# MIT-SPARK/Hydra-GNN

Hardware: AMD Instinct MI355X
Metric: scene-graphs/sec (fwd+bwd) MP3D hetero batch (higher is better)
Workload: dtype f32

## Files before the change

hydra-gnn_amd/csrc/gemm.hip:

```cpp
#include <algorithm>

#include "gemm_tile.h"

namespace hmp {

KT_DEFINE(gemm)

template <int ROWS, int BK>
using TileSide = TileSlots<256, ROWS, BK>;
template <int ROWS, int BK>
using TileRegs = StageRegs<TileSide<ROWS, BK>::NV>;

template <int ROWS, int BK>
__device__ __forceinline__ void tile_load_edge(TileRegs<ROWS, BK>& t, const float* __restrict__ p, int ld, int kcontig, int r0,
                                               int R, int n_real, int aug, int k0, int kend, int vec) {
  using S = TileSide<ROWS, BK>;
#pragma unroll
  for (int i = 0; i < S::NV; ++i) {
    float4 val = make_float4(0.f, 0.f, 0.f, 0.f);
    if (kcontig) {
      int r, k4;
      S::slot_rk(i, r, k4);
      const int gr = r0 + r, gk = k0 + k4;
      if (gr < R && gk < kend) {
// ... 405 lines not shown
    P.M = g.M; P.N = g.N; P.K = g.K; P.lda = g.lda; P.ldb = g.ldb; P.ldc = g.ldc; P.n_real = g.n_real; P.aug_ones = g.aug_ones;
    P.nslices = cdiv(g.N, TT_NS);
    int ks = (int)(512.0 * ((double)g.K * P.nslices / work_total) / P.nslices + 0.5);
    if (ks > GEMM_TALL_SLABS) ks = GEMM_TALL_SLABS;
    if (ks < 1) ks = 1;
    P.kchunk = g.kchunk = cdiv(cdiv(g.K, ks), TT_BK) * TT_BK;
    P.ksplit = g.ksplit = cdiv(g.K, P.kchunk);
    P.block_start = start;
    start += P.ksplit * P.nslices;
  }
  static const int rc = [] {
    return hipFuncSetAttribute(reinterpret_cast<const void*>(&gemm_tn_tall_kernel), hipFuncAttributeMaxDynamicSharedMemorySize,
                               2 * TT_STAGE * (int)sizeof(float)) == hipSuccess ? 0 : 1;
  }();
  HMP_CHECK_ARG(rc == 0, "gemm: could not raise the dynamic LDS limit of the tall weight-gradient kernel");
  hipLaunchKernelGGL(gemm_tn_tall_kernel, dim3(start), dim3(256), 2 * TT_STAGE * sizeof(float), st, tb);
  HMP_LAUNCH_CHECK();
  return HMP_OK;
}

int gemm_launch(GemmBatch& gb, bool want_split, int max_slabs, hipStream_t st) {
  HMP_CHECK_ARG(gb.n >= 0 && gb.n <= GEMM_MAX_PROB, "gemm: %d problems", gb.n);
  if (gemm_x3_takes(gb, want_split)) return gemm_x3_launch(gb, want_split, max_slabs, st);
  if (want_split) {
    GemmPeel tall;
    gemm_peel(gb, tall_takes, tall);
    if (tall.n_taken > 0) {
      HMP_TRY(tall_launch(gb, tall, st));
      return gemm_launch_rest(gb, tall, [&](GemmBatch& rest) { return gemm_launch(rest, want_split, max_slabs, st); });
    }
  }
  int64_t tiles64 = 0;
  double work = 0.0;
  int max_k = 0;
  for (int i = 0; i < gb.n; ++i) {
    const GemmProblem& p = gb.p[i];
    HMP_CHECK_ARG(p.M >= 0 && p.N >= 0 && p.K >= 0, "gemm: negative size");
    tiles64 += (int64_t)cdiv(p.M, 64) * cdiv(p.N, 64);
    work += (double)p.M * p.N * p.K;
    max_k = p.K > max_k ? p.K : max_k;
  }
  if (tiles64 >= 1024 || work >= 1e9) {
    int64_t tiles128 = 0;
    for (int i = 0; i < gb.n; ++i) tiles128 += (int64_t)cdiv(gb.p[i].M, 128) * cdiv(gb.p[i].N, 128);
    const bool big_ok = env_switch("HMP_GEMM_BIG") != '0';
    int min_n = 1 << 30;
    for (int i = 0; i < gb.n; ++i) min_n = gb.p[i].N < min_n ? gb.p[i].N : min_n;
    if (big_ok && min_n >= 256 && work >= 1e9 && (tiles128 >= 256 || (want_split && max_k >= 8192)))
      return launch_cfg<2, 2, 32, 2, 2>(gb, want_split, max_slabs, st);
    return launch_cfg<2, 2, 32>(gb, want_split, max_slabs, st);
  }
  if (max_k <= 64) return launch_cfg<1, 1, 64>(gb, want_split, max_slabs, st);
  return launch_cfg<1, 1, 128>(gb, want_split, max_slabs, st);
}

}

extern "C" int hmp_gemm_f32(const float* d_a, int32_t lda, int32_t trans_a, const float* d_b, int32_t ldb, int32_t trans_b,
                            float* d_c, int32_t ldc, int32_t M, int32_t N, int32_t K, void* stream) {
  using namespace hmp;
  HMP_CHECK_ARG(d_a && d_b && d_c, "hmp_gemm_f32: null pointer");
  HMP_CHECK_ARG(M >= 0 && N >= 0 && K >= 0, "hmp_gemm_f32: negative size");
  HMP_CHECK_ARG(lda >= (trans_a ? M : K) && ldb >= (trans_b ? K : N) && ldc >= N, "hmp_gemm_f32: leading dimension too small");
  GemmBatch gb;
  memset(&gb, 0, sizeof(gb));
  gb.n = 1;
  GemmProblem& p = gb.p[0];
  p.A = d_a; p.B = d_b; p.C = d_c;
  p.M = M; p.N = N; p.K = K;
  p.lda = lda; p.ldb = ldb; p.ldc = ldc;
  p.trans_a = trans_a; p.trans_b = trans_b;
  p.n_real = N;
  p.epi = EPI_NONE;
  if (M == 0 || N == 0) return HMP_OK;
  return gemm_launch(gb, false, 1, (hipStream_t)stream);
}

extern "C" int hmp_gemm_grouped(const hmp_gemm_desc* d, int32_t n, int32_t route, int32_t want_split, int32_t max_slabs,
                                int32_t* ksplit_out, void* stream) {
  using namespace hmp;
  static const bool have_device = hmp_device_count() > 0;
  HMP_CHECK_ARG(have_device, "hmp_gemm_grouped: no gfx950 device visible");
  HMP_CHECK_ARG((d || n == 0) && n >= 0 && n <= GEMM_MAX_PROB, "hmp_gemm_grouped: %d problems (at most %d)", n, GEMM_MAX_PROB);
  HMP_CHECK_ARG(route >= 0 && route <= 2 && max_slabs >= 1, "hmp_gemm_grouped: route %d, max_slabs %d", route, max_slabs);
  for (int i = 0; i < n; ++i) {
    const hmp_gemm_desc& q = d[i];
    HMP_CHECK_ARG(q.A && q.B && q.C, "hmp_gemm_grouped: null pointer (problem %d)", i);
    HMP_CHECK_ARG(q.M >= 0 && q.N >= 0 && q.K >= 0, "hmp_gemm_grouped: negative size (problem %d)", i);
    HMP_CHECK_ARG(q.n_real == q.N - (q.aug_ones ? 1 : 0) && q.n_real >= 0, "hmp_gemm_grouped: n_real %d, N %d, aug_ones %d (problem %d)",
                  q.n_real, q.N, q.aug_ones, i);
    HMP_CHECK_ARG(q.lda >= (q.trans_a ? q.M : q.K) && q.ldb >= (q.trans_b ? q.K : q.n_real) && q.ldc >= q.N,
                  "hmp_gemm_grouped: leading dimension too small (problem %d)", i);
    HMP_CHECK_ARG(q.epi == EPI_NONE || (q.epi == EPI_ACTMASK && q.H && q.ldh >= q.N), "hmp_gemm_grouped: epilogue (problem %d)", i);
    HMP_CHECK_ARG(!q.Cadd || q.ldadd >= q.N, "hmp_gemm_grouped: ldadd too small (problem %d)", i);
    HMP_CHECK_ARG(q.drop_p >= 0.f && q.drop_p < 1.f, "hmp_gemm_grouped: drop_p %g (problem %d)", (double)q.drop_p, i);
    HMP_CHECK_ARG(!want_split || q.M == 0 || q.slab_stride >= (int64_t)q.M * q.ldc, "hmp_gemm_grouped: slab_stride (problem %d)", i);
    HMP_CHECK_ARG(route == 1 || !(q.a_bf16 || q.b_bf16 || q.c_bf16 || q.h_bf16), "hmp_gemm_grouped: bf16 operands on route %d", route);
    HMP_CHECK_ARG(route != 2 || (q.trans_a && !q.trans_b && q.epi == EPI_NONE && !q.Cadd),
                  "hmp_gemm_grouped: the direct kernel takes the plain TN form only (problem %d)", i);
  }
  hipStream_t st = (hipStream_t)stream;
  if (route == 2) {
    TnBatch tb;
    memset(&tb, 0, sizeof(tb));
    tb.n = n;
    for (int i = 0; i < n; ++i) {
      const hmp_gemm_desc& q = d[i];
      TnProblem& P = tb.p[i];
      P.A = (const float*)q.A; P.B = (const float*)q.B; P.C = (float*)q.C; P.slab_stride = q.slab_stride;
      P.M = q.M; P.N = q.N; P.K = q.K; P.lda = q.lda; P.ldb = q.ldb; P.ldc = q.ldc;
      P.n_real = q.n_real; P.aug_ones = q.aug_ones;
    }
    int ok = 0;
    HMP_TRY(gemm_tn_direct_launch(tb, max_slabs, &ok, st));
    if (ksplit_out)
      for (int i = 0; i < n; ++i) ksplit_out[i] = ok ? tb.p[i].ksplit : 0;
    return HMP_OK;
  }
  GemmBatch gb;
  memset(&gb, 0, sizeof(gb));
  gb.n = n;
  for (int i = 0; i < n; ++i) {
    const hmp_gemm_desc& q = d[i];
    GemmProblem& p = gb.p[i];
    p.A = (const float*)q.A; p.B = (const float*)q.B; p.C = (float*)q.C; p.H = (const float*)q.H;
    p.a_bf16 = q.a_bf16; p.b_bf16 = q.b_bf16; p.c_bf16 = q.c_bf16; p.h_bf16 = q.h_bf16;
    p.slab_stride = q.slab_stride;
    p.M = q.M; p.N = q.N; p.K = q.K;
    p.lda = q.lda; p.ldb = q.ldb; p.ldc = q.ldc; p.ldh = q.ldh;
    p.trans_a = q.trans_a; p.trans_b = q.trans_b;
    p.n_real = q.n_real; p.aug_ones = q.aug_ones;
    p.epi = q.epi; p.act = q.act;
    p.drop_on = q.drop_p > 0.f ? 1 : 0;
    p.drop.thresh = drop_thresh(q.drop_p); p.drop.scale = 1.f / (1.f - q.drop_p);
    p.Cadd = q.Cadd; p.ldadd = q.ldadd;
  }
  const int rc = route == 0 ? gemm_launch(gb, want_split != 0, max_slabs, st) : gemm_bf16_launch(gb, want_split != 0, max_slabs, st);
  if (ksplit_out)
    for (int i = 0; i < n; ++i) ksplit_out[i] = gb.p[i].ksplit;
  return rc;
}
```

hydra-gnn_amd/csrc/gemm_direct.hip:

```cpp
#include "device_fns.h"

namespace hmp {

KT_DEFINE(gemmd)

typedef float f32x16 __attribute__((ext_vector_type(16)));

__device__ __forceinline__ void reduce4(f32x16& acc, float* red , int w, int lane, float (&out)[4]) {
#pragma unroll
  for (int i = 0; i < 16; ++i) red[(w * 16 + i) * 64 + lane] = acc[i];
  __syncthreads();
#pragma unroll
  for (int j = 0; j < 4; ++j) {
    const int i = 4 * w + j;
    out[j] = (red[(0 * 16 + i) * 64 + lane] + red[(1 * 16 + i) * 64 + lane]) + (red[(2 * 16 + i) * 64 + lane] + red[(3 * 16 + i) * 64 + lane]);
  }
}

constexpr int TN_MAXI = 24;

__global__ __launch_bounds__(256, 2) void gemm_tn_direct_kernel(const TnBatch tb) {
  __shared__ float red[4 * 16 * 64];
  const int blk = blockIdx.x;
  KT(8);
  karg_warm<(sizeof(TnBatch) + 63) / 64>(0, (int)sizeof(TnBatch));
  int pi = 0;
  while (pi + 1 < tb.n && blk >= tb.p[pi + 1].tile_start) ++pi;
  const TnProblem& P = tb.p[pi];
  const int local = blk - P.tile_start;
  const int z = local % P.ksplit, t = local / P.ksplit;
  const int tm = t / P.tiles_n, tn = t % P.tiles_n;
  const int m0 = tm * 32, n0 = tn * 32;
  const int lane = threadIdx.x & 63, w = threadIdx.x >> 6;
  const int r = lane & 31, h = lane >> 5;
  const int kbeg = z * P.kchunk, kend = min(P.K, kbeg + P.kchunk);
  const int n_steps = (kend - kbeg + 1) >> 1;
  const int per = (n_steps + 3) >> 2;
  const int s0 = w * per, s1 = min(n_steps, s0 + per);
  const int am = min(m0 + r, P.M - 1);
  const int bn = n0 + r;
  const bool b_real = bn < P.n_real;
  const bool b_one = P.aug_ones && bn == P.n_real;
  const int bnc = b_real ? bn : 0;
  f32x16 acc;
#pragma unroll
  for (int i = 0; i < 16; ++i) acc[i] = 0.f;
  for (int sb0 = s0; sb0 < s1; sb0 += TN_MAXI) {
    float av[TN_MAXI], bv[TN_MAXI];
#pragma unroll
    for (int i = 0; i < TN_MAXI; ++i) {
      const int k = kbeg + 2 * (sb0 + i) + h;
      const bool live = (sb0 + i < s1) && k < kend;
      const int kc = live ? k : kbeg;
      const float a = P.A[(int64_t)kc * P.lda + am];
      const float b = P.B[(int64_t)kc * P.ldb + bnc];
      av[i] = live ? a : 0.f;
      bv[i] = live ? (b_real ? b : (b_one ? 1.f : 0.f)) : 0.f;
    }
#pragma unroll
    for (int i = 0; i < TN_MAXI; ++i)
      if (sb0 + i < s1) acc = __builtin_amdgcn_mfma_f32_32x32x2f32(av[i], bv[i], acc, 0, 0, 0);
  }
  float out[4];
  reduce4(acc, red, w, lane, out);
  float* C = P.C + (int64_t)z * P.slab_stride;
  const int col = n0 + (lane & 31);
  if (col < P.N) {
#pragma unroll
    for (int j = 0; j < 4; ++j) {
      const int row = m0 + j + 8 * w + 4 * h;
      if (row < P.M) C[(int64_t)row * P.ldc + col] = out[j];
    }
  }
  KT(9);
}

int gemm_tn_direct_launch(TnBatch& tb, int max_slabs, int* ok, hipStream_t st) {
  int start = 0;
  *ok = 1;
  for (int i = 0; i < tb.n; ++i) {
    TnProblem& P = tb.p[i];
    P.tiles_m = cdiv(P.M, 32);
    P.tiles_n = cdiv(P.N, 32);
    const int trips = (P.tiles_m * P.tiles_n >= 512) ? 4 : 2;
    int ks = cdiv(P.K, 2 * 4 * TN_MAXI * trips);
    if (ks < 1) ks = 1;
    if (ks > max_slabs) { *ok = 0; return HMP_OK; }
    while (ks * 2 <= max_slabs && cdiv(P.K, ks * 2) >= 32 && P.tiles_m * P.tiles_n * ks < 256) ks *= 2;
    int kchunk = cdiv(cdiv(P.K, ks), 2) * 2;
    if (kchunk < 2) kchunk = 2;
    ks = P.K > 0 ? cdiv(P.K, kchunk) : 1;
    P.ksplit = ks;
    P.kchunk = kchunk;
    P.tile_start = start;
    start += P.tiles_m * P.tiles_n * ks;
  }
  tb.total_tiles = start;
  if (start == 0) return HMP_OK;
  hipLaunchKernelGGL(gemm_tn_direct_kernel, dim3(start), dim3(256), 0, st, tb);
  HMP_LAUNCH_CHECK();
  return HMP_OK;
}

}
```

hydra-gnn_amd/csrc/kernels.h:

```cpp
#pragma once
#include "common.h"

namespace hmp {

enum { EPI_NONE = 0, EPI_ACTMASK = 1 };

struct GemmProblem {
  const float* A;
  const float* B;
  float* C;
  const float* H;
  int c_bf16;
  int a_bf16;
  int b_bf16;
  int h_bf16;
  const float* A2;
  int lda2, a_split;
  int64_t slab_stride;
  int M, N, K;
  int lda, ldb, ldc, ldh;
  int trans_a;
  int trans_b;
  int n_real;
  int aug_ones;
// ... 83 lines not shown
    gb.p[s.rest_idx[i]].kchunk = s.rest.p[i].kchunk;
  }
  return rc;
}

struct XcdGrid {
  int groups, tiles_per_group;
};
inline XcdGrid xcd_set_grid(int per_cu, int n_slices, int n_tiles) {
  int sets = per_cu * device_cu_count() / (8 * n_slices);
  if (sets < 1) sets = 1;
  int groups = 8 * sets;
  if (groups > n_tiles) groups = ((n_tiles + 7) / 8) * 8;
  return {groups, cdiv(n_tiles, groups)};
}

int gemm_launch(GemmBatch& gb, bool want_split, int max_slabs, hipStream_t st);
int gemm_bf16_launch(GemmBatch& gb, bool want_split, int max_slabs, hipStream_t st);
bool gemm_x3_takes(const GemmBatch& gb, bool want_split);
bool gemm_x3_split_takes(const GemmProblem* ps, int n);
int gemm_x3_launch(GemmBatch& gb, bool want_split, int max_slabs, hipStream_t st);
bool gemm_bf16_dx_takes(const GemmProblem& p, bool want_split);
int gemm_bf16_dx_launch(const GemmProblem& p, hipStream_t st);
bool gemm_bf16_dw_takes(const GemmProblem& p, bool want_split);
int gemm_bf16_dw_launch(const GemmProblem& p, int max_slabs, int* n_slabs, hipStream_t st);

constexpr int FR_MAX_PROB = 4;
constexpr int FR_MAX_SEG = 6;
constexpr int FR_MAX_SRC = 6;
struct FrontSeg {
  int col0, rows, nsrc, ld;
  uint32_t off[FR_MAX_SRC];
};
struct FrontProb {
  const float* A;
  float* C;
  int lda, ldc, M, N, K;
  int n_seg, max_nsrc, vec;
  int blk_start, tiles_m, tiles_n;
  FrontSeg seg[FR_MAX_SEG];
};
struct FrontJob {
  const int64_t* ei;
  int E, n_src, n_dst;
  uint32_t rowptr, col, eid, t_rowptr, t_col, t_eid, tmp_in, tmp_out, pos_of_eid, degf;
  const int64_t *gp_dst, *gp_src, *gp_edge;
  int n_graphs;
};
struct PackSeg;
struct NetState;
struct FrontArgs {
  int gemm_blocks, plan_blocks, pack_blocks;
  int n_prob, n_jobs, need_tpos, plan_rc;
  const float* params;
  char* ws;
  int* status;
  const PackSeg* segs;
  const int2* pack_map;
  float* packed;
  int* step_ctr;
  int* step_mirror;
  int prob_start[FR_MAX_PROB];
  int part_start[2 * HMP_MAX_EDGE_TYPES + 1];
  int rows_per_part[2 * HMP_MAX_EDGE_TYPES];
  FrontJob job[HMP_MAX_EDGE_TYPES];
  FrontProb prob[FR_MAX_PROB];
};
int front_launch(FrontArgs& a, hipStream_t st);

struct TnProblem {
  const float* A;
  const float* B;
  float* C;
  int64_t slab_stride;
  int M, N, K, lda, ldb, ldc;
  int n_real, aug_ones;
  int ksplit, kchunk, tile_start, tiles_m, tiles_n;
};
struct TnBatch {
  int n, total_tiles;
  TnProblem p[GEMM_MAX_PROB];
};
int gemm_tn_direct_launch(TnBatch& tb, int max_slabs, int* ok, hipStream_t st);

struct PlanJob {
  const int64_t* ei;
  int64_t E;
  int n_src, n_dst;
  int *rowptr, *col, *eid, *t_rowptr, *t_col, *t_pos;
  float* degf;
  const int64_t *gp_dst, *gp_src, *gp_edge;
  int n_graphs;
  int *cnt_in, *cnt_out, *cur_in, *cur_out;
  int* flags;
  int *tmp_in, *tmp_out, *t_eid, *pos_of_eid;
  int *tmpc_in, *tmpc_out;
};
struct PlanBatch {
  int n;
  int need_tpos;
  int clear_first;
  int build_id;
  int* flags_all;
  int64_t edge_start[HMP_MAX_EDGE_TYPES + 1];
  int64_t row_start[2 * HMP_MAX_EDGE_TYPES + 1];
  PlanJob j[HMP_MAX_EDGE_TYPES];
};
size_t plan_scratch_ints(int64_t E, int n_src, int n_dst);
void plan_carve(PlanJob& job, int* scratch);
int plan_launch(PlanBatch& pb, int* d_status, hipStream_t st);
int plan_link_launch(PlanBatch& pb, hipStream_t st);

constexpr int AGG_MAX_IN = 6;
struct AggIn {
  const int* rowptr;
  const int* col;
  const float* z;
  int ldz, coff;
  int same_type;
  int n_src;
};
struct AggDst {
  int n_rows, F;
  float* out;
  int ldo;
  const float* zroot;
  int ldzr, roff;
  const float* bias;
  int n_in;
  int act;
  int drop_on;
  DropCfg drop;
  int block_start;
  const float* pw;
  float* pz;
  int pldw, pldz, pncols, pK;
  const int64_t* ce_labels;
  int64_t ce_ignored;
  int ce_classes, ce_ldg;
  float* ce_grad;
  float* ce_row_lv;
  const uint8_t* ce_mask;
  int ce_tail;
  int win_in;
  int tile_rows;
  AggIn in[AGG_MAX_IN];
};
struct AggArgs {
  int n;
  int total_blocks;
  int mean;
  int xcd;
  int zb16;
  int hb16;
  NetState* state;
  int bstart[HMP_MAX_NODE_TYPES];
  AggDst d[HMP_MAX_NODE_TYPES];
};
int agg_fwd_launch(AggArgs& a, hipStream_t st);
int agg_proj_fwd_launch(AggArgs& a, hipStream_t st);

struct TAggOut {
  const int* t_rowptr;
  const int* t_col;
  const int* rowptr;
  const float* degf;
// ... 263 lines not shown
```

hydra-gnn_amd/csrc/net.hip:

```cpp
#include <cstdlib>
#include <vector>

#include "plan_small.h"

using namespace hmp;

namespace {

struct ConvLayout {
  int coff;
  int asoff, adoff;
  int H, C, Cp;
  int64_t vedge_off;
  int64_t vslab_off;
  bool wd_is_src;
  float *smax, *sden, *alpha_drop, *dlogit, *dlogit_orig;
  bool agg_first;
  int aoff, ld_m;
  int64_t wc_off, cslab_off;
  float *mrows, *dmrows;
};

struct LayerLayout {
  int kind;
  int n_live;
  int live[HMP_MAX_CONVS];
  ConvLayout conv[HMP_MAX_CONVS];
  int n_in[HMP_MAX_NODE_TYPES];
  bool reads[HMP_MAX_NODE_TYPES];
  int aggf_of_src[HMP_MAX_NODE_TYPES];
  int ncols[HMP_MAX_NODE_TYPES];
  int roff[HMP_MAX_NODE_TYPES];
  int64_t wp_off[HMP_MAX_NODE_TYPES];
  int ldw[HMP_MAX_NODE_TYPES];
  int64_t wpt_off[HMP_MAX_NODE_TYPES];
  int ldt[HMP_MAX_NODE_TYPES];
  int64_t bias_off[HMP_MAX_NODE_TYPES];
  int64_t slab_off[HMP_MAX_NODE_TYPES];
  int lddw[HMP_MAX_NODE_TYPES];
  int64_t bslab_off[HMP_MAX_NODE_TYPES];
  GatLayerS* d_gat;
  GatLayerS h_gat;
};

constexpr int MAX_SLABS = 192;
static_assert(MAX_SLABS >= GEMM_TALL_SLABS, "the slab buffer must hold what the tall weight-gradient kernel may write");
constexpr int TN_DIRECT_SLABS = 16;

struct ProfRec {
  int cls;
  hipEvent_t a, b;
};

}

struct EnvSwitches {
  bool plan_sliced = true;
  bool front = true;
  bool z16 = true;
  bool h16 = true;
  bool rootcopy = false;
  bool tn_direct = true;
  bool bf16_all = false;
};

struct StepCall {
  int training = 0;
  uint64_t seed = 0;
  uint32_t rng_step = 0;
  int* d_step = nullptr;
  const int64_t* ce_labels = nullptr;
  const hmp_head_targets* tgt = nullptr;
  int64_t ce_ignored = 0;
  AdamFuse adam = {};
  bool fin_loss = false;
  int fin_rows = 0;
  bool aux_g_ready = false;
  int head_blocks = 0;
  bool ce_done = false;
  bool tail_done[2] = {false, false};
  bool adam_done = false;
};

struct hmp_net {
  hmp_net_spec spec;
  EnvSwitches env;
  int T, ET, L;
  int dim[HMP_MAX_LAYERS + 1][HMP_MAX_NODE_TYPES];
  int ld[HMP_MAX_LAYERS + 1][HMP_MAX_NODE_TYPES];
  LayerLayout lay[HMP_MAX_LAYERS];
  int64_t packed_floats, slab_floats;
  int out_dim, out_ld;
  bool any_gat = false;
  bool pass0[HMP_MAX_NODE_TYPES] = {false};

  PackSeg* d_pack_segs = nullptr;
  int n_pack = 0;
  int64_t pack_rows = 0;
  GradSeg* d_grad_segs = nullptr;
  int n_grad = 0;
  int64_t grad_elems = 0;
  int max_pack_rows = 0;
  int64_t max_grad_elems = 0;
  SegBlocks pack_sb, grad_sb;
  int2* d_pack_map = nullptr;
  int n_pack_blocks16 = 0;
  char* ws_base = nullptr;
  size_t ws_bytes = 0;
  float* degf[HMP_MAX_EDGE_TYPES];
  bool any_agg_first = false;
  int* d_iota = nullptr;
  float* d_ones = nullptr;
  float* d_sadd = nullptr;
  int iota_cap = 0;
  int64_t sadd_floats = 0;
  float* d_row_lv = nullptr;

  bool bound = false;
  int cap_nodes[HMP_MAX_NODE_TYPES];
  int64_t cap_edges[HMP_MAX_EDGE_TYPES];
  NetState* d_state = nullptr;
  hmp_plan plan[HMP_MAX_EDGE_TYPES];
  int* plan_scratch[HMP_MAX_EDGE_TYPES];
  float* d_packed = nullptr;
  float* d_slabs = nullptr;
  float* H[HMP_MAX_LAYERS + 1][HMP_MAX_NODE_TYPES];
  float* G[HMP_MAX_LAYERS + 1][HMP_MAX_NODE_TYPES];
  bool h16[HMP_MAX_LAYERS + 1][HMP_MAX_NODE_TYPES] = {};
  float* Z[HMP_MAX_LAYERS][HMP_MAX_NODE_TYPES];
  float* dZ[HMP_MAX_LAYERS][HMP_MAX_NODE_TYPES];
  float* d_out = nullptr;
  float* d_gout = nullptr;
  int cap_out = 0;

  bool have_fwd = false;
  bool plan_ok = false;
  hmp_batch batch;
  int training = 0;
  uint64_t seed = 0;
  uint32_t rng_step = 0;
  GradReduceDyn dyn;
  StepCall call;

  int compute_bf16 = 0;
  int fuse_mode = -1;
  bool fuse_now = false;
  bool reuse_plan = false;
  bool has_heads = false;
  hmp_linear_heads heads = {};
  int64_t head_slab_off = 0, head_slab_stride = 0;
  int head_ld_slab = 0;
  bool has_pools = false;
  int head_pool[2] = {-1, -1};
  float* d_dpool[2] = {nullptr, nullptr};

  bool prof = false;
  std::vector<ProfRec> recs;
};

namespace {

void read_env(hmp_net* n) {
  EnvSwitches e;
  e.plan_sliced = env_switch("HMP_PLAN_SLICED") != '0';
  e.front = env_switch("HMP_FRONT") != '0';
  e.z16 = env_switch("HMP_Z16") != '0';
  e.h16 = env_switch("HMP_H16") != '0';
  e.rootcopy = env_switch("HMP_ROOTCOPY") == '1';
  e.tn_direct = env_switch("HMP_TN") != '0';
  e.bf16_all = env_switch("HMP_BF16_ALL") == '1';
  n->env = e;
}

inline int fpad(int f) { return align4(f); }

inline int head_type(const hmp_net* n, int h) { return h == 0 ? n->spec.readout_type : n->spec.aux_readout_type; }
inline int label_type(const hmp_net* n, int h) {
  return n->head_pool[h] >= 0 ? n->spec.edge_dst[n->head_pool[h]] : head_type(n, h);
}

int build_layout(hmp_net* n) {
  const hmp_net_spec& S = n->spec;
  n->T = S.n_node_types; n->ET = S.n_edge_types; n->L = S.n_layers;
  HMP_CHECK_ARG(n->T >= 1 && n->T <= HMP_MAX_NODE_TYPES, "net: n_node_types %d", n->T);
  HMP_CHECK_ARG(n->ET >= 1 && n->ET <= HMP_MAX_EDGE_TYPES, "net: n_edge_types %d", n->ET);
  HMP_CHECK_ARG(n->L >= 1 && n->L <= HMP_MAX_LAYERS, "net: n_layers %d", n->L);
  HMP_CHECK_ARG(S.readout_type >= 0 && S.readout_type < n->T, "net: readout_type");
  HMP_CHECK_ARG(S.pool_edge_type >= -1 && S.pool_edge_type < n->ET, "net: pool_edge_type");
  HMP_CHECK_ARG(S.aux_readout_type >= -1 && S.aux_readout_type < n->T && S.aux_readout_type != S.readout_type &&
                    (S.aux_readout_type < 0 || S.pool_edge_type < 0),
                "net: aux_readout_type (a second node type, not with a pooled output)");
  for (int e = 0; e < n->ET; ++e)
    HMP_CHECK_ARG(S.edge_src[e] >= 0 && S.edge_src[e] < n->T && S.edge_dst[e] >= 0 && S.edge_dst[e] < n->T, "net: edge type %d endpoints", e);
  for (int t = 0; t < n->T; ++t) {
    n->dim[0][t] = S.in_dim[t];
    n->ld[0][t] = 0;
  }
  int64_t packed = 0, slabs = 0;
  for (int l = 0; l < n->L; ++l) {
    const hmp_layer_spec& Ls = S.layers[l];
    LayerLayout& Y = n->lay[l];
    HMP_CHECK_ARG(Ls.n_convs >= 1 && Ls.n_convs <= HMP_MAX_CONVS, "net: layer %d has %d convs", l, Ls.n_convs);
    Y.kind = Ls.convs[0].kind;
    Y.d_gat = nullptr;
    HMP_CHECK_ARG(Y.kind == HMP_CONV_SAGE || Y.kind == HMP_CONV_GAT, "net: layer %d: unknown conv kind %d", l, Y.kind);
    HMP_CHECK_ARG(Ls.group_mean == 0 || Y.kind == HMP_CONV_GAT, "net: HeteroConv aggr=mean is only supported for GAT layers");
    for (int t = 0; t < n->T; ++t) {
      n->dim[l + 1][t] = Ls.out_dim[t];
      n->ld[l + 1][t] = fpad(Ls.out_dim[t]);
      if (Ls.passthrough[t]) {
        HMP_CHECK_ARG(l == 0 && n->L > 1, "net: passthrough node types are supported on the first layer only");
        HMP_CHECK_ARG(Ls.out_dim[t] == S.in_dim[t], "net: passthrough type %d must keep its input width", t);
        n->pass0[t] = true;
      }
      Y.ncols[t] = 0;
      Y.roff[t] = -1;
      Y.n_in[t] = 0;
      Y.reads[t] = false;
      Y.aggf_of_src[t] = -1;
    }
    Y.n_live = 0;
    int n_outgoing[HMP_MAX_NODE_TYPES] = {0};
    for (int c = 0; c < Ls.n_convs; ++c) {
      const hmp_conv_spec& C = Ls.convs[c];
      ConvLayout& Q = Y.conv[c];
      memset(&Q, 0, sizeof(Q));
      HMP_CHECK_ARG(C.kind == Y.kind, "net: layer %d mixes conv kinds", l);
      HMP_CHECK_ARG(C.edge_type >= 0 && C.edge_type < n->ET, "net: conv edge_type");
      HMP_CHECK_ARG(C.src == S.edge_src[C.edge_type] && C.dst == S.edge_dst[C.edge_type], "net: conv endpoints disagree with edge type");
      HMP_CHECK_ARG(n->dim[l][C.src] > 0 && n->dim[l][C.dst] > 0, "net: layer %d conv %d reads a node type with no features", l, c);
      if (Y.kind == HMP_CONV_SAGE) {
        HMP_CHECK_ARG(C.f_out == Ls.out_dim[C.dst], "net: SAGE f_out must equal the layer's out_dim of the destination type");
      } else {
        HMP_CHECK_ARG(gat_shape_ok(C.heads, C.f_out), "net: GAT heads %d / channels %d unsupported (at most %d channels per head, at most %d heads above 256 channels)",
                      C.heads, C.f_out, GAT_CMAX, GAT_WIDE_HMAX);
        HMP_CHECK_ARG(Ls.out_dim[C.dst] == (C.concat ? C.heads * C.f_out : C.f_out), "net: GAT out_dim mismatch on layer %d conv %d", l, c);
        HMP_CHECK_ARG(C.edge_dim >= 0 && C.edge_dim <= GAT_MAX_EDIM, "net: GAT edge_dim %d > %d", C.edge_dim, GAT_MAX_EDIM);
        HMP_CHECK_ARG(!(C.edge_dim > 0 && C.fill_mean && C.self_loops), "net: fill_value='mean' with edge attributes is not supported (the reference passes zeros)");
        HMP_CHECK_ARG(!C.self_loops || C.src == C.dst, "net: self loops need src == dst (the reference sets add_self_loops = (src == dst))");
      }
      HMP_CHECK_ARG(!C.agg_first || (Y.kind == HMP_CONV_SAGE && C.src != C.dst), "net: agg_first is for SAGE convs between two node types");
      if (!C.active) continue;
      Y.live[Y.n_live++] = c;
      ++Y.n_in[C.dst];
      const bool aggf = C.agg_first != 0;
      ++n_outgoing[aggf ? C.dst : C.src];
      HMP_CHECK_ARG(Y.n_in[C.dst] <= AGG_MAX_IN && n_outgoing[C.src] <= AGG_MAX_IN && n_outgoing[C.dst] <= AGG_MAX_IN,
                    "net: more than %d convs share a node type", AGG_MAX_IN);
      Y.reads[C.src] = Y.reads[C.dst] = true;
      if (Y.kind == HMP_CONV_SAGE) {
        HMP_CHECK_ARG(C.w0 >= 0 && C.b0 >= 0 && C.w1 >= 0, "net: SAGE conv needs lin_l.weight, lin_l.bias, lin_r.weight");
        if (aggf) {
// ... 1166 lines not shown
        gb = l > 0 && g16[l];
        HMP_TRY(seg_mean_rows_t_launch(Q.dmrows, Q.ld_m, fpad(n->dim[l][s]), T.P->d_t_rowptr, T.P->d_t_col, T.degf, b->n_nodes[s],
                                       masked ? (const void*)n->H[l][s] : nullptr, n->ld[l][s], n->h16[l][s] ? 1 : 0, act, drop_on ? 1 : 0,
                                       drop_on ? 1.f / (1.f - Lp->dropout) : 1.f, dst, l > 0 ? n->ld[l][s] : b->ldx[s], gb ? 1 : 0, st));
      }
    }
    {
      auto add = [&](int sid, const GemmProblem& p) {
        n->dyn.slab_stride[sid] = (int)p.slab_stride;
        wids.push_back(sid);
        wps.push_back(p);
      };
      for (int s = 0; s < n->T; ++s) {
        if (Y.ncols[s] == 0 || b->n_nodes[s] == 0) continue;
        GemmProblem p;
        memset(&p, 0, sizeof(p));
        p.A = n->dZ[l][s]; p.lda = Y.ncols[s]; p.trans_a = 1;
        p.a_bf16 = dz16 ? 1 : 0;
        if (rootless && Y.roff[s] >= 0) { int ldg; p.A2 = g_of(s, ldg); p.lda2 = ldg; p.a_split = Y.roff[s]; }
        p.B = h_ptr(n, l, s); p.ldb = h_ld(n, l, s); p.trans_b = 0;
        p.b_bf16 = n->h16[l][s] ? 1 : 0;
        p.C = n->d_slabs + Y.slab_off[s]; p.ldc = Y.lddw[s];
        p.slab_stride = (int64_t)Y.ncols[s] * Y.lddw[s];
        p.M = Y.ncols[s]; p.N = n->dim[l][s] + 1; p.K = b->n_nodes[s];
        p.n_real = n->dim[l][s]; p.aug_ones = 1;
        add(slab_id_w(l, s), p);
      }
      for (int i = 0; i < Y.n_live; ++i) {
        const int c = Y.live[i];
        if (!aggf_live(c)) continue;
        const hmp_conv_spec& C = Ls.convs[c];
        const ConvLayout& Q = Y.conv[c];
        GemmProblem p;
        memset(&p, 0, sizeof(p));
        p.A = dz_at(C.dst, Q.aoff); p.lda = Y.ncols[C.dst]; p.trans_a = 1; p.a_bf16 = dz16 ? 1 : 0;
        p.B = Q.mrows; p.ldb = Q.ld_m; p.trans_b = 0;
        p.C = n->d_slabs + Q.cslab_off; p.ldc = Y.lddw[C.src];
        p.slab_stride = (int64_t)fpad(C.f_out) * Y.lddw[C.src];
        p.M = fpad(C.f_out); p.N = n->dim[l][C.src]; p.K = b->n_nodes[C.dst];
        p.n_real = p.N; p.aug_ones = 0;
        add(slab_id_v(l, c), p);
      }
      if (Y.kind == HMP_CONV_GAT) {
        for (int t = 0; t < n->T; ++t) {
          if (Y.n_in[t] == 0 || b->n_nodes[t] == 0) continue;
          int ldg;
          const float* g = g_of(t, ldg);
          GemmProblem p;
          memset(&p, 0, sizeof(p));
          p.A = g; p.lda = ldg; p.trans_a = 1;
          p.B = g; p.ldb = ldg; p.trans_b = 0;
          p.C = n->d_slabs + Y.bslab_off[t]; p.ldc = 4;
          p.slab_stride = (int64_t)fpad(Ls.out_dim[t]) * 4;
          p.M = Ls.out_dim[t]; p.N = 1; p.K = b->n_nodes[t];
          p.n_real = 0; p.aug_ones = 1;
          add(slab_id_b(l, t), p);
        }
        for (int i = 0; i < Y.n_live; ++i) {
          const int c = Y.live[i];
          const hmp_conv_spec& C = Ls.convs[c];
          if (C.edge_dim == 0 || b->n_edges[C.edge_type] == 0) continue;
          GemmProblem p;
          memset(&p, 0, sizeof(p));
          p.A = b->d_edge_attr[C.edge_type]; p.lda = C.edge_dim; p.trans_a = 1;
          p.B = Y.conv[c].dlogit_orig; p.ldb = GAT_HMAX; p.trans_b = 0;
          p.C = n->d_slabs + Y.conv[c].vslab_off; p.ldc = GAT_HMAX;
          p.slab_stride = GAT_MAX_EDIM * GAT_HMAX;
          p.M = C.edge_dim; p.N = C.heads; p.K = (int)b->n_edges[C.edge_type];
          p.n_real = C.heads;
          add(slab_id_v(l, c), p);
        }
      }
    }
  }
  {
    Scope sc(n, KC_GEMM_BWD, st);
    std::vector<int> ks;
    bool direct = n->fuse_now;
    if (direct) {
      if (!n->env.tn_direct) direct = false;
      if (direct && !n->compute_bf16 && !wps.empty() && gemm_x3_split_takes(wps.data(), (int)wps.size())) direct = false;
      for (size_t i = 0; i < wps.size() && direct; ++i)
        if (wps[i].K > TN_DIRECT_SLABS * 384 || wps[i].b_bf16 || wps[i].a_bf16) direct = false;
      for (size_t base = 0; base < wps.size() && direct; base += GEMM_MAX_PROB) {
        TnBatch tb;
        memset(&tb, 0, sizeof(tb));
        const size_t cnt = (wps.size() - base) < (size_t)GEMM_MAX_PROB ? (wps.size() - base) : (size_t)GEMM_MAX_PROB;
        for (size_t i = 0; i < cnt; ++i) {
          const GemmProblem& g = wps[base + i];
          TnProblem& P = tb.p[tb.n++];
          P.A = g.A; P.B = g.B; P.C = g.C; P.slab_stride = g.slab_stride;
          P.M = g.M; P.N = g.N; P.K = g.K; P.lda = g.lda; P.ldb = g.ldb; P.ldc = g.ldc;
          P.n_real = g.n_real; P.aug_ones = g.aug_ones;
        }
        int ok = 0;
        HMP_TRY(gemm_tn_direct_launch(tb, TN_DIRECT_SLABS, &ok, st));
        HMP_CHECK_ARG(ok, "net: weight-gradient problem too deep for the direct kernel after the size check");
        for (size_t i = 0; i < cnt; ++i) ks.push_back(tb.p[i].ksplit);
      }
    }
    if (!direct) HMP_TRY(gemm_many(n, wps, true, st, &ks));
    for (size_t i = 0; i < wids.size(); ++i) n->dyn.n_slabs[wids[i]] = (unsigned char)ks[i];
  }
  {
    Scope sc(n, KC_GRAD_REDUCE, st);
    const int64_t na = n->spec.n_active_params;
    AdamFuse af = n->call.adam;
    af.on = (af.on && fin_early && !n->any_gat) ? 1 : 0;
    n->call.adam_done = af.on != 0;
    HMP_TRY(grad_reduce_launch(n->d_grad_segs, n->grad_sb, n->dyn, n->d_slabs, d_params, d_grads,
                               n->call.fin_loss ? n->d_row_lv : nullptr, n->call.fin_rows > 0 ? n->call.fin_rows : b->n_out, d_grads + na, n->d_state,
                               af, st));
    n->call.fin_loss = false;
  }
  return HMP_OK;
}

struct StepGuard {
  hmp_net* n;
  StepGuard(hmp_net* net, int training = 0, uint64_t seed = 0, uint32_t rng_step = 0, int* d_step = nullptr) : n(net) {
    read_env(n);
    n->call.training = training; n->call.seed = seed; n->call.rng_step = rng_step;
    n->call.d_step = d_step;
  }
  ~StepGuard() { n->call = StepCall(); }
  StepGuard(const StepGuard&) = delete;
  StepGuard& operator=(const StepGuard&) = delete;
};

int plain_forward(hmp_net* n, const hmp_batch* b, const float* d_params, hipStream_t st, int training = 0, uint64_t seed = 0,
                  uint32_t rng_step = 0) {
  StepGuard guard(n, training, seed, rng_step);
  return forward_impl(n, b, d_params, st);
}

}

extern "C" int hmp_net_create(const hmp_net_spec* spec, hmp_net** out) {
  HMP_CHECK_ARG(spec && out, "hmp_net_create: null argument");
  HMP_CHECK_ARG(hmp_device_count() > 0, "hmp_net_create: no gfx950 device visible");
  hmp_net* n = new hmp_net;
  n->spec = *spec;
  int r = build_layout(n);
  if (r == HMP_OK) r = build_tables(n);
  if (r == HMP_OK) {
    if (hipMalloc(&n->d_state, 256) != hipSuccess || hipMemset(n->d_state, 0, 256) != hipSuccess) {
      snprintf(err_buf(), 512, "hmp_net_create: device allocation of the net state failed");
      r = HMP_E_HIP;
    }
  }
  if (r == HMP_OK) {
    const int fz = env_switch("HMP_FUSE");
    n->fuse_mode = fz < 0 ? -1 : fz == '1' ? 1 : 0;
  }
  if (r != HMP_OK) {
    hmp_net_destroy(n);
    return r;
  }
  *out = n;
  return HMP_OK;
}

extern "C" void hmp_net_destroy(hmp_net* n) {
  if (!n) return;
  for (auto& r : n->recs) { (void)hipEventDestroy(r.a); (void)hipEventDestroy(r.b); }
  if (n->d_state) (void)hipFree(n->d_state);
  if (n->d_pack_segs) (void)hipFree(n->d_pack_segs);
  if (n->d_pack_map) (void)hipFree(n->d_pack_map);
  if (n->d_grad_segs) (void)hipFree(n->d_grad_segs);
  for (int l = 0; l < HMP_MAX_LAYERS; ++l)
    if (l < n->L && n->lay[l].d_gat) (void)hipFree(n->lay[l].d_gat);
  delete n;
}

extern "C" size_t hmp_net_workspace_bytes(const hmp_net* net, const int32_t* cap_nodes, const int64_t* cap_edges) {
  if (!net || !cap_nodes || !cap_edges) return 0;
  hmp_net tmp = *net;
  tmp.recs.clear();
  return carve(&tmp, nullptr, cap_nodes, cap_edges);
}

// ... 538 lines not shown
```

Baseline: 376,100.

## Add 64x64 paired-tile direct TN kernel for weight-gradient GEMMs

Adds a weight-gradient TN GEMM kernel in which each lane loads float2 pairs of A and B and feeds four 32x32 MFMA accumulators, covering a 64x64 output tile per block. This improves operand reuse and vectorises the loads. The augmented-ones column is computed as a running sum of A instead of a dedicated MFMA lane. By default it is used only when the planner reports deep K chunks and alignment allows, with an environment override. The cost is four times the accumulator registers, twice the shared memory for the reduction, and fewer blocks per problem.

```diff
diff --git a/hydra-gnn_amd/csrc/gemm.hip b/hydra-gnn_amd/csrc/gemm.hip
--- a/hydra-gnn_amd/csrc/gemm.hip
+++ b/hydra-gnn_amd/csrc/gemm.hip
@@ -511,7 +511,7 @@
   static const bool have_device = hmp_device_count() > 0;
   HMP_CHECK_ARG(have_device, "hmp_gemm_grouped: no gfx950 device visible");
   HMP_CHECK_ARG((d || n == 0) && n >= 0 && n <= GEMM_MAX_PROB, "hmp_gemm_grouped: %d problems (at most %d)", n, GEMM_MAX_PROB);
-  HMP_CHECK_ARG(route >= 0 && route <= 2 && max_slabs >= 1, "hmp_gemm_grouped: route %d, max_slabs %d", route, max_slabs);
+  HMP_CHECK_ARG(route >= 0 && route <= 3 && max_slabs >= 1, "hmp_gemm_grouped: route %d, max_slabs %d", route, max_slabs);
   for (int i = 0; i < n; ++i) {
     const hmp_gemm_desc& q = d[i];
     HMP_CHECK_ARG(q.A && q.B && q.C, "hmp_gemm_grouped: null pointer (problem %d)", i);
@@ -525,11 +525,11 @@
     HMP_CHECK_ARG(q.drop_p >= 0.f && q.drop_p < 1.f, "hmp_gemm_grouped: drop_p %g (problem %d)", (double)q.drop_p, i);
     HMP_CHECK_ARG(!want_split || q.M == 0 || q.slab_stride >= (int64_t)q.M * q.ldc, "hmp_gemm_grouped: slab_stride (problem %d)", i);
     HMP_CHECK_ARG(route == 1 || !(q.a_bf16 || q.b_bf16 || q.c_bf16 || q.h_bf16), "hmp_gemm_grouped: bf16 operands on route %d", route);
-    HMP_CHECK_ARG(route != 2 || (q.trans_a && !q.trans_b && q.epi == EPI_NONE && !q.Cadd),
-                  "hmp_gemm_grouped: the direct kernel takes the plain TN form only (problem %d)", i);
+    HMP_CHECK_ARG(route < 2 || (q.trans_a && !q.trans_b && q.epi == EPI_NONE && !q.Cadd),
+                  "hmp_gemm_grouped: the direct kernels take the plain TN form only (problem %d)", i);
   }
   hipStream_t st = (hipStream_t)stream;
-  if (route == 2) {
+  if (route >= 2) {
     TnBatch tb;
     memset(&tb, 0, sizeof(tb));
     tb.n = n;
@@ -541,7 +541,8 @@
       P.n_real = q.n_real; P.aug_ones = q.aug_ones;
     }
     int ok = 0;
-    HMP_TRY(gemm_tn_direct_launch(tb, max_slabs, &ok, st));
+    if (route == 2) HMP_TRY(gemm_tn_direct_launch(tb, max_slabs, &ok, st));
+    else HMP_TRY(gemm_tn_pair_launch(tb, max_slabs, &ok, st));
     if (ksplit_out)
       for (int i = 0; i < n; ++i) ksplit_out[i] = ok ? tb.p[i].ksplit : 0;
     return HMP_OK;
diff --git a/hydra-gnn_amd/csrc/gemm_direct.hip b/hydra-gnn_amd/csrc/gemm_direct.hip
--- a/hydra-gnn_amd/csrc/gemm_direct.hip
+++ b/hydra-gnn_amd/csrc/gemm_direct.hip
@@ -1,3 +1,5 @@
+#include <algorithm>
+
 #include "device_fns.h"
 
 namespace hmp {
@@ -102,4 +104,184 @@
   return HMP_OK;
 }
 
-}
+typedef float f32x2 __attribute__((ext_vector_type(2)));
+
+template <int STEPS, bool PAIR_B>
+__device__ __forceinline__ void pair_trip(const float* __restrict__ A, const float* __restrict__ B, int lda, int ldb, int kbeg,
+                                          int kend, int sb0, int s1, int h, int am, int bn, bool b0, bool b1,
+                                          f32x16 (&acc)[2][2], float& sa0, float& sa1) {
+  f32x2 av[STEPS], bv[STEPS];
+#pragma unroll
+  for (int i = 0; i < STEPS; ++i) {
+    const int k = kbeg + 2 * (sb0 + i) + h;
+    const bool live = (sb0 + i < s1) && k < kend;
+    const int kc = live ? k : kbeg;
+    const f32x2 a = *(const f32x2*)(A + (int64_t)kc * lda + am);
+    const float* pb = B + (int64_t)kc * ldb + bn;
+    f32x2 b;
+    if (PAIR_B) {
+      b = *(const f32x2*)pb;
+    } else {
+      b.x = pb[0];
+      b.y = pb[b1 ? 1 : 0];
+    }
+    av[i].x = live ? a.x : 0.f;
+    av[i].y = live ? a.y : 0.f;
+    bv[i].x = (live && b0) ? b.x : 0.f;
+    bv[i].y = (live && b1) ? b.y : 0.f;
+  }
+#pragma unroll
+  for (int i = 0; i < STEPS; ++i)
+    if (sb0 + i < s1) {
+      acc[0][0] = __builtin_amdgcn_mfma_f32_32x32x2f32(av[i].x, bv[i].x, acc[0][0], 0, 0, 0);
+      acc[0][1] = __builtin_amdgcn_mfma_f32_32x32x2f32(av[i].x, bv[i].y, acc[0][1], 0, 0, 0);
+      acc[1][0] = __builtin_amdgcn_mfma_f32_32x32x2f32(av[i].y, bv[i].x, acc[1][0], 0, 0, 0);
+      acc[1][1] = __builtin_amdgcn_mfma_f32_32x32x2f32(av[i].y, bv[i].y, acc[1][1], 0, 0, 0);
+      sa0 += av[i].x;
+      sa1 += av[i].y;
+    }
+}
+
+constexpr int TN_PAIR_EDGE = 16;
+
+__global__ __launch_bounds__(256, 2) void gemm_tn_pair_kernel(const TnBatch tb) {
+  __shared__ float red[2][4 * 16 * 64];
+  __shared__ float ones[4][2][64];
+  const int blk = blockIdx.x;
+  KT(8);
+  karg_warm<(sizeof(TnBatch) + 63) / 64>(0, (int)sizeof(TnBatch));
+  int pi = 0;
+  while (pi + 1 < tb.n && blk >= tb.p[pi + 1].tile_start) ++pi;
+  const TnProblem& P = tb.p[pi];
+  const int local = blk - P.tile_start;
+  const int z = local % P.ksplit, t = local / P.ksplit;
+  const int tm = t / P.tiles_n, tn = t % P.tiles_n;
+  const int m0 = tm * 64, n0 = tn * 64;
+  const int lane = threadIdx.x & 63, w = threadIdx.x >> 6;
+  const int r = lane & 31, h = lane >> 5;
+  const int kbeg = z * P.kchunk, kend = min(P.K, kbeg + P.kchunk);
+  const int n_steps = (kend - kbeg + 1) >> 1;
+  const int per = (n_steps + 3) >> 2;
+  const int s0 = w * per, s1 = min(n_steps, s0 + per);
+  const int am = min(m0 + 2 * r, P.M - 2);
+  const bool b0 = n0 + 2 * r < P.n_real, b1 = n0 + 2 * r + 1 < P.n_real;
+  const int bn = b0 ? n0 + 2 * r : 0;
+  const bool straddle = (P.n_real & 1) && n0 + 64 > P.n_real;
+  f32x16 acc[2][2];
+#pragma unroll
+  for (int q = 0; q < 4; ++q)
+#pragma unroll
+    for (int i = 0; i < 16; ++i) acc[q >> 1][q & 1][i] = 0.f;
+  float sa0 = 0.f, sa1 = 0.f;
+  if (!straddle) {
+    for (int sb0 = s0; sb0 < s1; sb0 += TN_MAXI)
+      pair_trip<TN_MAXI, true>(P.A, P.B, P.lda, P.ldb, kbeg, kend, sb0, s1, h, am, bn, b0, b1, acc, sa0, sa1);
+  } else {
+    for (int sb0 = s0; sb0 < s1; sb0 += TN_PAIR_EDGE)
+      pair_trip<TN_PAIR_EDGE, false>(P.A, P.B, P.lda, P.ldb, kbeg, kend, sb0, s1, h, am, bn, b0, b1, acc, sa0, sa1);
+  }
+  const bool do_ones = P.aug_ones && tn == 0;
+  if (do_ones) {
+    ones[w][h][2 * r] = sa0;
+    ones[w][h][2 * r + 1] = sa1;
+  }
+  float* C = P.C + (int64_t)z * P.slab_stride;
+  const bool cvec = !(P.ldc & 1) && !(P.slab_stride & 1) && !((uintptr_t)P.C & 7);
+  const int col = n0 + 2 * r;
+#pragma unroll
+  for (int ja = 0; ja < 2; ++ja) {
+    if (ja) __syncthreads();
+#pragma unroll
+    for (int jb = 0; jb < 2; ++jb)
+#pragma unroll
+      for (int i = 0; i < 16; ++i) red[jb][(w * 16 + i) * 64 + lane] = acc[ja][jb][i];
+    __syncthreads();
+#pragma unroll
+    for (int j = 0; j < 4; ++j) {
+      const int i = 4 * w + j;
+      float o[2];
+#pragma unroll
+      for (int jb = 0; jb < 2; ++jb)
+        o[jb] = (red[jb][(0 * 16 + i) * 64 + lane] + red[jb][(1 * 16 + i) * 64 + lane]) +
+                (red[jb][(2 * 16 + i) * 64 + lane] + red[jb][(3 * 16 + i) * 64 + lane]);
+      const int row = m0 + 2 * (j + 8 * w + 4 * h) + ja;
+      if (row < P.M) {
+        float* c = C + (int64_t)row * P.ldc + col;
+        if (cvec && b1) {
+          f32x2 v;
+          v.x = o[0]; v.y = o[1];
+          *(f32x2*)c = v;
+        } else {
+          if (b0) c[0] = o[0];
+          if (b1) c[1] = o[1];
+        }
+      }
+    }
+    if (ja == 0 && do_ones && w == 0) {
+      const int row = m0 + lane;
+      const float s = ((ones[0][0][lane] + ones[0][1][lane]) + (ones[1][0][lane] + ones[1][1][lane])) +
+                      ((ones[2][0][lane] + ones[2][1][lane]) + (ones[3][0][lane] + ones[3][1][lane]));
+      if (row < P.M) C[(int64_t)row * P.ldc + P.n_real] = s;
+    }
+  }
+  KT(9);
+}
+
+bool gemm_tn_pair_takes(const TnBatch& tb) {
+  for (int i = 0; i < tb.n; ++i) {
+    const TnProblem& P = tb.p[i];
+    if (P.M == 0) continue;
+    if ((P.M & 1) || (P.lda & 1) || (P.ldb & 1) || P.n_real < 1) return false;
+    if (((uintptr_t)P.A & 7) || ((uintptr_t)P.B & 7)) return false;
+  }
+  return true;
+}
+
+bool gemm_tn_pair_plan(TnBatch& tb, int max_slabs) {
+  constexpr int TRIP = 2 * 4 * TN_MAXI;
+  bool deep = false;
+  for (int trips = 1;; ++trips) {
+    int total = 0;
+    for (int i = 0; i < tb.n; ++i) {
+      TnProblem& P = tb.p[i];
+      P.tiles_m = cdiv(P.M, 64);
+      P.tiles_n = cdiv(P.n_real, 64);
+      int ks = cdiv(P.K, TRIP * trips);
+      ks = ks < 1 ? 1 : (ks > max_slabs ? max_slabs : ks);
+      int kchunk = cdiv(cdiv(P.K, ks), 2) * 2;
+      if (kchunk < 2) kchunk = 2;
+      P.kchunk = kchunk;
+      P.ksplit = P.K > 0 ? cdiv(P.K, kchunk) : 1;
+      total += P.tiles_m * P.tiles_n * P.ksplit;
+      if (P.M > 0 && kchunk > TRIP + TRIP / 2) deep = true;
+    }
+    if (total <= 512 || trips == 8) break;
+  }
+  return deep;
+}
+
+int gemm_tn_pair_launch(TnBatch& tb, int max_slabs, int* ok, hipStream_t st) {
+  *ok = gemm_tn_pair_takes(tb) ? 1 : 0;
+  if (!*ok) return HMP_OK;
+  gemm_tn_pair_plan(tb, max_slabs);
+  int order[GEMM_MAX_PROB];
+  for (int i = 0; i < tb.n; ++i) order[i] = i;
+  std::stable_sort(order, order + tb.n, [&](int a, int b) { return tb.p[a].kchunk > tb.p[b].kchunk; });
+  TnBatch sb;
+  memset(&sb, 0, sizeof(sb));
+  sb.n = tb.n;
+  int start = 0;
+  for (int j = 0; j < tb.n; ++j) {
+    TnProblem& P = tb.p[order[j]];
+    P.tile_start = start;
+    start += P.tiles_m * P.tiles_n * P.ksplit;
+    sb.p[j] = P;
+  }
+  tb.total_tiles = sb.total_tiles = start;
+  if (start == 0) return HMP_OK;
+  hipLaunchKernelGGL(gemm_tn_pair_kernel, dim3(start), dim3(256), 0, st, sb);
+  HMP_LAUNCH_CHECK();
+  return HMP_OK;
+}
+
+}
diff --git a/hydra-gnn_amd/csrc/kernels.h b/hydra-gnn_amd/csrc/kernels.h
--- a/hydra-gnn_amd/csrc/kernels.h
+++ b/hydra-gnn_amd/csrc/kernels.h
@@ -189,6 +189,9 @@
   TnProblem p[GEMM_MAX_PROB];
 };
 int gemm_tn_direct_launch(TnBatch& tb, int max_slabs, int* ok, hipStream_t st);
+bool gemm_tn_pair_takes(const TnBatch& tb);
+bool gemm_tn_pair_plan(TnBatch& tb, int max_slabs);
+int gemm_tn_pair_launch(TnBatch& tb, int max_slabs, int* ok, hipStream_t st);
 
 struct PlanJob {
   const int64_t* ei;
diff --git a/hydra-gnn_amd/csrc/net.hip b/hydra-gnn_amd/csrc/net.hip
--- a/hydra-gnn_amd/csrc/net.hip
+++ b/hydra-gnn_amd/csrc/net.hip
@@ -61,6 +61,7 @@
   bool h16 = true;
   bool rootcopy = false;
   bool tn_direct = true;
+  int tn_pair = -1;
   bool bf16_all = false;
 };
 
@@ -168,6 +169,7 @@
   e.h16 = env_switch("HMP_H16") != '0';
   e.rootcopy = env_switch("HMP_ROOTCOPY") == '1';
   e.tn_direct = env_switch("HMP_TN") != '0';
+  e.tn_pair = env_switch("HMP_TN_PAIR") == '0' ? 0 : (env_switch("HMP_TN_PAIR") == '1' ? 1 : -1);
   e.bf16_all = env_switch("HMP_BF16_ALL") == '1';
   n->env = e;
 }
@@ -1500,6 +1502,7 @@
       if (direct && !n->compute_bf16 && !wps.empty() && gemm_x3_split_takes(wps.data(), (int)wps.size())) direct = false;
       for (size_t i = 0; i < wps.size() && direct; ++i)
         if (wps[i].K > TN_DIRECT_SLABS * 384 || wps[i].b_bf16 || wps[i].a_bf16) direct = false;
+      std::vector<TnBatch> tbs;
       for (size_t base = 0; base < wps.size() && direct; base += GEMM_MAX_PROB) {
         TnBatch tb;
         memset(&tb, 0, sizeof(tb));
@@ -1511,10 +1514,22 @@
           P.M = g.M; P.N = g.N; P.K = g.K; P.lda = g.lda; P.ldb = g.ldb; P.ldc = g.ldc;
           P.n_real = g.n_real; P.aug_ones = g.aug_ones;
         }
+        tbs.push_back(tb);
+      }
+      bool pair = direct && n->env.tn_pair != 0;
+      for (size_t j = 0; j < tbs.size() && pair; ++j) pair = gemm_tn_pair_takes(tbs[j]);
+      if (pair && n->env.tn_pair < 0) {
+        bool deep = false;
+        for (size_t j = 0; j < tbs.size(); ++j) deep = gemm_tn_pair_plan(tbs[j], TN_DIRECT_SLABS) || deep;
+        pair = deep;
+      }
+      for (size_t j = 0; j < tbs.size() && direct; ++j) {
+        TnBatch& tb = tbs[j];
         int ok = 0;
-        HMP_TRY(gemm_tn_direct_launch(tb, TN_DIRECT_SLABS, &ok, st));
-        HMP_CHECK_ARG(ok, "net: weight-gradient problem too deep for the direct kernel after the size check");
-        for (size_t i = 0; i < cnt; ++i) ks.push_back(tb.p[i].ksplit);
+        if (pair) HMP_TRY(gemm_tn_pair_launch(tb, TN_DIRECT_SLABS, &ok, st));
+        else HMP_TRY(gemm_tn_direct_launch(tb, TN_DIRECT_SLABS, &ok, st));
+        HMP_CHECK_ARG(ok, "net: weight-gradient problem refused by the direct kernel after the size check");
+        for (int i = 0; i < tb.n; ++i) ks.push_back(tb.p[i].ksplit);
       }
     }
     if (!direct) HMP_TRY(gemm_many(n, wps, true, st, &ks));
```

After: 372,100. 0.989x the previous value.
